# giech/usrp_nfc

Hardware: AMD Instinct MI355X
Metric: IQ Msamples/s -> decoded bits (2 Msps stream) (higher is better)
Workload: dtype f32 envelope / f64 window sums / u8 symbols; 1 GPU; configs[1]: Miller-only decode, synthetic IQ @2 Msps; input_kind=fc32 IQ, 8 B/sample (envelope computed in the kernel), samples_per_gpu=100000000, parallelism=time-chunk x1, edges_per_gpu=6627699, symbols_reader=3971547, symbols_tag=0, packets=101186, boundary_redos=0, exchange=none, stepping=sync, in_flight=1

## Files before the change

usrp_nfc_amd/csrc/decode.hip.h:

```cpp
#pragma once
#include <hip/hip_runtime.h>
#include <stdint.h>

#include "../../include/nfc_amd.h"
#include "scan.hip.h"

namespace nfc {

struct DecTables {
    const uint4 *mil_map;
    const uint2 *man_map;
    const uint16_t *mil_step;
    const uint16_t *man_step;
    int32_t nd;
    int32_t reader, tag;
    const uint2 *qmil_map;
    const uint16_t *qmil_step;
    uint32_t q_rep[2];
    uint32_t canon[4];
    int32_t q_ok;
};
__device__ __forceinline__ uint32_t byte_of(const uint32_t *w, uint32_t i) { return (w[i >> 2] >> (8u * (i & 3u))) & 0xFFu; }

struct DecCarry {
    int32_t mil_state, man_state;
    int32_t pkt_started[2];
    uint32_t pending[2];
};

constexpr int DEC_ITEMS = 16;
#ifndef NFC_DEC_GROUPS
#define NFC_DEC_GROUPS 2
#endif
constexpr int DEC_GROUPS = NFC_DEC_GROUPS;
constexpr int DEC_PER_THREAD = DEC_ITEMS * DEC_GROUPS;
constexpr int DEC_TILE = SCAN_BLOCK * DEC_PER_THREAD;
constexpr int DEC_LDS_ROWS = 512;
inline size_t dec_num_tiles(size_t n) { return (n + DEC_TILE - 1) / DEC_TILE; }

enum DecLdsUser { DEC_LDS_SPEC = 0, DEC_LDS_REDUCE = 1, DEC_LDS_APPLY = 2 };
inline size_t dec_table_bytes(DecLdsUser k, const DecTables &T) {
    const size_t rows = 4 * (size_t)T.nd, nr = T.reader ? 1 : 0, nt = T.tag ? 1 : 0;
    if (rows > (size_t)DEC_LDS_ROWS) return 0;
    switch (k) {
    case DEC_LDS_SPEC: return (nr + nt) * (rows * 16 + (rows + 1) * 8);
    case DEC_LDS_REDUCE: return nr * rows * 16 + nt * rows * 8;
    default: return nr * rows * 32 + nt * rows * 16;
    }
}

__device__ __forceinline__ void load_codes(const uint16_t *ecode, size_t base, size_t n, uint32_t (&c)[8]) {
    if (base + DEC_ITEMS <= n) {
        const uint4 a = *(const uint4 *)(ecode + base), b = *(const uint4 *)(ecode + base + 8);
        c[0] = a.x; c[1] = a.y; c[2] = a.z; c[3] = a.w;
        c[4] = b.x; c[5] = b.y; c[6] = b.z; c[7] = b.w;
    } else {
#pragma unroll
        for (int k = 0; k < 8; k++) {
            const size_t i = base + 2 * k;
            c[k] = (i < n ? (uint32_t)ecode[i] : 0u) | (i + 1 < n ? (uint32_t)ecode[i + 1] << 16 : 0u);
        }
    }
}
__device__ __forceinline__ void load_bytes16(const uint8_t *p, size_t base, size_t n, uint32_t fill, uint32_t (&w)[4]) {
    if (base + 16 <= n) {
        const uint4 a = *(const uint4 *)(p + base);
        w[0] = a.x; w[1] = a.y; w[2] = a.z; w[3] = a.w;
    } else {
#pragma unroll
        for (int k = 0; k < 4; k++) {
            uint32_t v = 0;
#pragma unroll
            for (int q = 0; q < 4; q++) {
                const size_t i = base + 4 * k + q;
                v |= (i < n ? (uint32_t)p[i] : fill) << (8 * q);
            }
            w[k] = v;
        }
    }
}

constexpr uint32_t PM_STOP = 0u, PM_START = 1u, PM_ID = 2u;
constexpr uint32_t FA_DB = 4u, FA_DC = 8u;
struct FrameAgg {
    uint32_t cnt[2];
    uint32_t nb[2], nc[2];
    uint32_t fl[2];
};
struct FrameAggOp {
    using T = FrameAgg;
    static __host__ __device__ __forceinline__ T identity() { return T{{0u, 0u}, {0u, 0u}, {0u, 0u}, {PM_ID, PM_ID}}; }
    static __device__ __forceinline__ T op(const T &a, const T &b) {
        T r;
#pragma unroll
        for (int t = 0; t < 2; t++) {
            const uint32_t ma = a.fl[t] & 3u, mb = b.fl[t] & 3u;
            const bool into_stopped = ma == PM_STOP;
            r.cnt[t] = a.cnt[t] + b.cnt[t];
            r.nb[t] = a.nb[t] + b.nb[t] - (into_stopped ? (b.fl[t] >> 2) & 1u : 0u);
            r.nc[t] = a.nc[t] + b.nc[t] - (into_stopped ? (b.fl[t] >> 3) & 1u : 0u);
            r.fl[t] = (mb == PM_ID ? ma : mb) | ((ma == PM_ID ? b.fl[t] : a.fl[t]) & (FA_DB | FA_DC));
        }
        return r;
    }
    static __device__ __forceinline__ T shfl_up(const T &v, int d) {
        T r;
#pragma unroll
        for (int t = 0; t < 2; t++) {
            r.cnt[t] = (uint32_t)__shfl_up((int)v.cnt[t], d, 64);
            r.nb[t] = (uint32_t)__shfl_up((int)v.nb[t], d, 64);
            r.nc[t] = (uint32_t)__shfl_up((int)v.nc[t], d, 64);
            r.fl[t] = (uint32_t)__shfl_up((int)v.fl[t], d, 64);
        }
        return r;
    }
};
struct FramePk {
    uint32_t a[2], b[2];
};
struct FramePkOp {
    using T = FramePk;
    static __device__ __forceinline__ T pack(const FrameAgg &f) {
        return T{{f.cnt[0] | (f.nb[0] << 16), f.cnt[1] | (f.nb[1] << 16)}, {f.nc[0] | (f.fl[0] << 16), f.nc[1] | (f.fl[1] << 16)}};
    }
    static __device__ __forceinline__ FrameAgg unpack(const T &p) {
        return FrameAgg{{p.a[0] & 0xFFFFu, p.a[1] & 0xFFFFu}, {p.a[0] >> 16, p.a[1] >> 16}, {p.b[0] & 0xFFFFu, p.b[1] & 0xFFFFu}, {p.b[0] >> 16, p.b[1] >> 16}};
    }
    static __device__ __forceinline__ T identity() { return T{{0u, 0u}, {PM_ID << 16, PM_ID << 16}}; }
    static __device__ __forceinline__ T op(const T &x, const T &y) {
        T r;
#pragma unroll
        for (int t = 0; t < 2; t++) {
            const uint32_t ma = (x.b[t] >> 16) & 3u, mb = (y.b[t] >> 16) & 3u;
            const uint32_t stopped = ma == PM_STOP ? 1u : 0u;
            r.a[t] = x.a[t] + y.a[t] - ((stopped & (y.b[t] >> 18)) << 16);
            const uint32_t nc = (x.b[t] & 0xFFFFu) + (y.b[t] & 0xFFFFu) - (stopped & (y.b[t] >> 19));
            const uint32_t fl = (mb == PM_ID ? ma : mb) | (((ma == PM_ID ? y.b[t] : x.b[t]) >> 16) & (FA_DB | FA_DC));
            r.b[t] = nc | (fl << 16);
        }
        return r;
    }
};
__device__ __forceinline__ uint32_t pm_apply(uint32_t fl, uint32_t started) { return (fl & 3u) == PM_ID ? started : (fl & 3u); }
__device__ __forceinline__ uint32_t fa_bits(const FrameAgg &a, int t, uint32_t started) { return a.nb[t] - (started ? 0u : (a.fl[t] >> 2) & 1u); }
__device__ __forceinline__ uint32_t fa_closes(const FrameAgg &a, int t, uint32_t started) { return a.nc[t] - (started ? 0u : (a.fl[t] >> 3) & 1u); }
__device__ __forceinline__ uint32_t start_bit_of(int type) { return type == 0 ? 1u : 0u; }
__device__ __forceinline__ uint32_t transpose_pairs(uint32_t m0, uint32_t m1, uint32_t m2, uint32_t m3) {
    uint32_t x = m0 | (m1 << 2) | (m2 << 4) | (m3 << 6);
    uint32_t t = (x ^ (x >> 6)) & 0x00CC00CCu;
    x ^= t ^ (t << 6);
    t = (x ^ (x >> 12)) & 0x0000F0F0u;
    x ^= t ^ (t << 12);
    return x;
}
struct SlotMasks {
    uint32_t V[2], ST[2], SA[2];
};
template <int DECS = 3>
__device__ __forceinline__ SlotMasks slot_masks(const uint32_t (&ow)[4]) {
    constexpr uint32_t M = 0x01010101u;
    uint32_t V1[4], ST1[4], SA1[4], V0[4], ST0[4], SA0[4];
#pragma unroll
    for (int i = 0; i < 4; i++) {
        const uint32_t w = ow[i];
        const uint32_t b0 = w & M, b1 = (w >> 1) & M;
        const uint32_t v0 = b0 & b1;
        const uint32_t v1e = b0 ^ b1;
        const uint32_t v1o = b1 & ~b0;
        const uint32_t c2 = (w >> 2) & M, hi0 = ((w >> 3) | (w >> 4)) & M;
        const uint32_t c5 = (w >> 5) & M, hi1 = ((w >> 6) | (w >> 7)) & M;
        const uint32_t z0 = M ^ (c2 | hi0), z1 = M ^ (c5 | hi1);
        const uint32_t o0 = c2 & ~hi0;
        V1[i] = v1e | (v1o << 1);
        ST1[i] = (hi0 & v1e) | ((hi1 & v1o) << 1);
        SA1[i] = (z0 & v1e) | ((z1 & v1o) << 1);
        V0[i] = v0;
        ST0[i] = hi0 & v0;
        SA0[i] = o0 & v0;
    }
    SlotMasks m{{0u, 0u}, {0u, 0u}, {0u, 0u}};
    if (DECS & 2) {
        m.V[0] = transpose_pairs(V0[0], V0[1], V0[2], V0[3]);
        m.ST[0] = transpose_pairs(ST0[0], ST0[1], ST0[2], ST0[3]);
        m.SA[0] = transpose_pairs(SA0[0], SA0[1], SA0[2], SA0[3]);
    }
    if (DECS & 1) {
        m.V[1] = transpose_pairs(V1[0], V1[1], V1[2], V1[3]);
        m.ST[1] = transpose_pairs(ST1[0], ST1[1], ST1[2], ST1[3]);
        m.SA[1] = transpose_pairs(SA1[0], SA1[1], SA1[2], SA1[3]);
    }
    return m;
}
__device__ __forceinline__ uint32_t started_before(const SlotMasks &m, int t, uint32_t started) {
    const uint32_t x = m.SA[t] | ~(m.ST[t] | m.SA[t]), y = m.SA[t];
    return (x + y + started) ^ x ^ y;
}
template <int DECS = 3>
__device__ __forceinline__ FrameAgg frame_agg_of(const uint32_t (&ow)[4]) {
    const SlotMasks m = slot_masks<DECS>(ow);
    FrameAgg a;
#pragma unroll
    for (int t = 0; t < 2; t++) {
        const uint32_t nonid = m.ST[t] | m.SA[t];
        const uint32_t before = started_before(m, t, 1u);
        const uint32_t appended = m.V[t] & ~m.ST[t] & (before | ~m.SA[t]);
        const uint32_t closes = m.ST[t] & before;
        const uint32_t first = nonid & (0u - nonid);
        a.cnt[t] = (uint32_t)__popc(m.V[t]);
        a.nb[t] = (uint32_t)__popc(appended);
        a.nc[t] = (uint32_t)__popc(closes);
        a.fl[t] = nonid == 0u ? PM_ID
                              : ((m.ST[t] > m.SA[t] ? PM_STOP : PM_START) | ((first & m.SA[t]) ? FA_DB : 0u) | ((first & m.ST[t]) ? FA_DC : 0u));
    }
    return a;
}
__device__ __forceinline__ uint32_t compress32(uint32_t x, uint32_t m) {
    x &= m;
    uint32_t mk = ~m << 1;
#pragma unroll
    for (int i = 0; i < 5; i++) {
        uint32_t mp = mk ^ (mk << 1);
        mp ^= mp << 2;
        mp ^= mp << 4;
        mp ^= mp << 8;
        mp ^= mp << 16;
        const uint32_t mv = mp & m;
        m = (m ^ mv) | (mv >> (1 << i));
        const uint32_t t = x & mv;
        x = (x ^ t) | (t >> (1 << i));
        mk &= ~mp;
    }
    return x;
}
__device__ __forceinline__ uint32_t symbol_low_bits(const uint32_t (&ow)[4]) {
    constexpr uint32_t M = 0x01010101u;
    uint32_t b[4];
#pragma unroll
    for (int i = 0; i < 4; i++) b[i] = ((ow[i] >> 2) & M) | (((ow[i] >> 5) & M) << 1);
    return transpose_pairs(b[0], b[1], b[2], b[3]);
}

struct PktCnt {
    uint64_t v[2];
};

struct ZeroJob {
    uint32_t *p[2];
    uint32_t n[2];
};
__device__ __forceinline__ void zero_words(const ZeroJob &Z) {
#pragma unroll
    for (int t = 0; t < 2; t++)
        for (uint32_t i = blockIdx.x * blockDim.x + threadIdx.x; i < Z.n[t]; i += gridDim.x * blockDim.x) Z.p[t][i] = 0u;
}

template <bool LDS>
__global__ __launch_bounds__(SCAN_BLOCK) void k_dec_reduce(const uint16_t *ecode, size_t n, const uint32_t *n_dev, DecTables T,
                                                          DecMaps *partials, DecMaps *aggs, ZeroJob Z) {
    zero_words(Z);
    if (n_dev) n = min(n, (size_t)*n_dev);
    if ((size_t)blockIdx.x * DEC_TILE >= n) return;
    TP_DECL();
    extern __shared__ __attribute__((aligned(16))) unsigned char s_dec_tab[];
    uint4 *const s_mil = (uint4 *)s_dec_tab;
    uint2 *const s_man = (uint2 *)(s_mil + (LDS && T.reader ? 4 * T.nd : 0));
    __shared__ DecMaps lds[SCAN_WAVES];
    if (LDS) {
        const int rows = 4 * T.nd;
        for (int i = threadIdx.x; i < rows; i += SCAN_BLOCK) {
            if (T.reader) s_mil[i] = T.mil_map[i];
            if (T.tag) s_man[i] = T.man_map[i];
        }
        __syncthreads();
    }
    const size_t tid = (size_t)blockIdx.x * SCAN_BLOCK + threadIdx.x;
    uint32_t c[DEC_GROUPS][8];
#pragma unroll
    for (int g = 0; g < DEC_GROUPS; g++) load_codes(ecode, tid * DEC_PER_THREAD + DEC_ITEMS * g, n, c[g]);
    TP_MARK();
    DecMaps agg = ComposeDec::identity();
#pragma unroll
    for (int g = 0; g < DEC_GROUPS; g++) {
#pragma unroll
        for (int k = 0; k < DEC_ITEMS; k++) {
            const uint32_t code = (c[g][k >> 1] >> (16 * (k & 1))) & 0xFFFFu;
            const uint32_t li = code & 0x3FFFu, route = code >> 14;
            if (route == 2u && T.reader) {
                const uint4 v = LDS ? s_mil[li] : T.mil_map[li];
#pragma unroll
                for (int q = 0; q < 4; q++) agg.mil[q] = lookup16x4(v.x, v.y, v.z, v.w, agg.mil[q]);
            } else if (route == 1u && T.tag) {
                const uint2 v = LDS ? s_man[li] : T.man_map[li];
                agg.man[0] = __builtin_amdgcn_perm(v.y, v.x, agg.man[0]);
                agg.man[1] = __builtin_amdgcn_perm(v.y, v.x, agg.man[1]);
            }
        }
    }
    TP_MARK();
    aggs[tid] = agg;
    DecMaps total;
    (void)block_exclusive<ComposeDec>(agg, lds, total);
    if (threadIdx.x == 0) partials[blockIdx.x] = total;
    TP_DONE(1);
}

template <bool LDS>
__global__ __launch_bounds__(SCAN_BLOCK) void k_dec_apply(const uint16_t *ecode, size_t n, const uint32_t *n_dev, DecTables T,
                                                         const DecMaps *partials, const DecMaps *aggs, uint32_t state0,
                                                         uint8_t *outw, FrameAgg *frame_aggs, FramePk *thread_aggs, bool own_prefix, DecMaps *total_out) {
    if (n_dev) n = min(n, (size_t)*n_dev);
    if (own_prefix && n == 0 && blockIdx.x == 0 && threadIdx.x == 0) *total_out = ComposeDec::identity();
    if ((size_t)blockIdx.x * DEC_TILE >= n) return;
    TP_DECL();
    extern __shared__ __attribute__((aligned(16))) unsigned char s_dec_tab[];
    uint16_t *const s_mil = (uint16_t *)s_dec_tab;
    uint16_t *const s_man = s_mil + (LDS && T.reader ? 4 * T.nd * 16 : 0);
    __shared__ DecMaps lds[SCAN_WAVES];
    __shared__ FramePk lds2[SCAN_WAVES];
    const DecMaps pre = own_prefix ? tile_prefix<ComposeDec, SCAN_BLOCK>(partials, blockIdx.x, lds) : partials[blockIdx.x];
    TP_MARK();
    if (LDS) {
        const int rows = 4 * T.nd;
        if (T.reader)
            for (int i = threadIdx.x; i < rows * 2; i += SCAN_BLOCK) ((uint4 *)s_mil)[i] = ((const uint4 *)T.mil_step)[i];
        if (T.tag)
            for (int i = threadIdx.x; i < rows; i += SCAN_BLOCK) ((uint4 *)s_man)[i] = ((const uint4 *)T.man_step)[i];
    }
    const size_t tid = (size_t)blockIdx.x * SCAN_BLOCK + threadIdx.x;
    const size_t base = tid * DEC_PER_THREAD;
    uint32_t c[DEC_GROUPS][8];
#pragma unroll
    for (int g = 0; g < DEC_GROUPS; g++) load_codes(ecode, base + DEC_ITEMS * g, n, c[g]);
    DecMaps total;
    const DecMaps excl = block_exclusive<ComposeDec>(aggs[tid], lds, total);
    if (own_prefix && threadIdx.x == 0 && ((size_t)blockIdx.x + 1) * DEC_TILE >= n) *total_out = ComposeDec::op(pre, total);
    uint32_t st = ComposeDec::step(ComposeDec::op(pre, excl), state0);
    TP_MARK();
    const uint16_t *mil = LDS ? s_mil : T.mil_step;
    const uint16_t *man = LDS ? s_man : T.man_step;
    FramePk mine = FramePkOp::identity();
#pragma unroll
    for (int g = 0; g < DEC_GROUPS; g++) {
        uint32_t ow[4] = {0u, 0u, 0u, 0u};
#pragma unroll
        for (int k = 0; k < DEC_ITEMS; k++) {
            const uint32_t code = (c[g][k >> 1] >> (16 * (k & 1))) & 0xFFFFu;
            const uint32_t li = code & 0x3FFFu, route = code >> 14;
            uint32_t w = 0;
            if (route == 2u && T.reader) {
                const uint32_t e = mil[li * 16u + (st & 15u)];
                w = e >> 8;
                st = (st & ~15u) | (e & 15u);
            } else if (route == 1u && T.tag) {
                const uint32_t e = man[li * 8u + ((st >> 4) & 7u)];
                const uint32_t m = e >> 8;
                w = (m & 3u) ? ((m & 0xFCu) | 3u) : 0u;
                st = (st & 15u) | ((e & 15u) << 4);
            }
            ow[k >> 2] |= w << (8 * (k & 3));
        }
        const size_t gb = base + (size_t)DEC_ITEMS * g;
        if (gb < n) *(uint4 *)(outw + gb) = make_uint4(ow[0], ow[1], ow[2], ow[3]);
        mine = FramePkOp::op(mine, FramePkOp::pack(frame_agg_of(ow)));
    }
    TP_MARK();
    FramePk total_fa;
    *(uint4 *)(thread_aggs + tid) = make_uint4(mine.a[0], mine.a[1], mine.b[0], mine.b[1]);
    (void)block_exclusive<FramePkOp>(mine, lds2, total_fa);
    if (threadIdx.x == 0) frame_aggs[blockIdx.x] = FramePkOp::unpack(total_fa);
    TP_DONE(2);
}

constexpr int FW_WORDS = DEC_TILE * 2 / 32 + 4;
constexpr uint32_t ST_CLOSES = 512 * DEC_GROUPS;
struct TileStage {
    uint32_t *bits[2];
    uint32_t *close_bit[2];
    uint64_t *close_idx[2];
    uint32_t *drop_bit[2];
    FrameAgg *own;
    const uint32_t *epos;
    uint64_t g0;
    const uint64_t *idx64;
};
__device__ __forceinline__ void bitcopy_or(uint32_t *dst, uint32_t dst_bit, const uint32_t *src, uint32_t src_bit, uint32_t nbits, uint32_t cap_bits) {
    if (!nbits) return;
    const uint32_t w0 = dst_bit >> 5, nw = ((dst_bit & 31u) + nbits + 31u) >> 5, capw = (cap_bits + 31u) >> 5;
    for (uint32_t j = threadIdx.x; j < nw; j += blockDim.x) {
        if (w0 + j >= capw) break;
        const uint32_t lo = max(dst_bit, (w0 + j) << 5), hi = min(dst_bit + nbits, (w0 + j + 1u) << 5);
        const uint32_t sb = src_bit + (lo - dst_bit), k = sb & 31u;
        const uint32_t a = src[sb >> 5], b = k ? src[(sb >> 5) + 1u] : 0u;
        uint32_t v = (a >> k) | (k ? b << (32u - k) : 0u);
        const uint32_t cnt = hi - lo;
        if (cnt < 32u) v &= (1u << cnt) - 1u;
        v <<= (lo & 31u);
        if (v) atomicOr(dst + w0 + j, v);
    }
}

struct QMaps {
    uint32_t mil[2];
    uint32_t man[2];
};
struct ComposeQ {
    using T = QMaps;
    static __host__ __device__ __forceinline__ T identity() { return T{{0x03020100u, 0x07060504u}, {0x03020100u, 0x07060504u}}; }
    static __device__ __forceinline__ T op(const T &a, const T &b) {
        return T{{__builtin_amdgcn_perm(b.mil[1], b.mil[0], a.mil[0]), __builtin_amdgcn_perm(b.mil[1], b.mil[0], a.mil[1])},
                 {__builtin_amdgcn_perm(b.man[1], b.man[0], a.man[0]), __builtin_amdgcn_perm(b.man[1], b.man[0], a.man[1])}};
    }
    static __device__ __forceinline__ uint32_t step(const T &m, uint32_t st) {
        const uint32_t a = __builtin_amdgcn_perm(m.mil[1], m.mil[0], st & 7u) & 15u;
        const uint32_t b = __builtin_amdgcn_perm(m.man[1], m.man[0], (st >> 4) & 7u) & 15u;
        return a | (b << 4);
    }
};
struct DecSpec {
    QMaps map;
    uint32_t s_in;
    uint32_t needs;
    uint32_t pad[2];
};
static_assert(sizeof(DecSpec) == 32, "two 16-byte loads");
__device__ __forceinline__ bool map8_constant(const uint32_t (&m)[2]) { return m[0] == m[1] && m[0] == (m[0] & 0xFFu) * 0x01010101u; }
constexpr int DEC_RUNIN_MAX = 8;
static_assert(DEC_GROUPS >= 1 && DEC_GROUPS <= 2, "NFC_DEC_GROUPS: a thread's packed bits are accumulated in 64 bits (32 slots per group)");
static_assert(DEC_RUNIN_MAX * SCAN_BLOCK <= DEC_TILE, "the longest run-in fits inside the tile before");
template <bool LDS, int DECS>
__global__ __launch_bounds__(SCAN_BLOCK) void k_dec_spec(const uint16_t *ecode, size_t n, const uint32_t *n_dev, DecTables T, uint32_t state0, int runin_per_thread,
                                                        uint8_t *outw, FrameAgg *frame_aggs, DecSpec *spec, ZeroJob Z, TileStage S) {
    constexpr bool RD = (DECS & 1) != 0, TG = (DECS & 2) != 0;
    zero_words(Z);
    if (n_dev) n = min(n, (size_t)*n_dev);
    if ((size_t)blockIdx.x * DEC_TILE >= n) return;
    TP_DECL();
    extern __shared__ __attribute__((aligned(16))) unsigned char s_dec_tab[];
    const int trows = LDS ? 4 * T.nd : 0;
    uint16_t *const s_mil = (uint16_t *)s_dec_tab, *const s_man = s_mil + (RD ? trows * 8 : 0);
    uint2 *const s_milmap = (uint2 *)(s_man + (TG ? trows * 8 : 0)), *const s_manmap = s_milmap + (LDS && RD ? trows + 1 : 0);
    __shared__ QMaps lds[SCAN_WAVES];
    __shared__ FramePk lds2[SCAN_WAVES];
    __shared__ uint32_t s_needs;
    __shared__ uint32_t s_bits[2][FW_WORDS];
    __shared__ uint32_t s_drop[2];
    for (int i = threadIdx.x; i < 2 * FW_WORDS; i += SCAN_BLOCK) (&s_bits[0][0])[i] = 0u;
    if (threadIdx.x < 2) s_drop[threadIdx.x] = 0xFFFFFFFFu;
    const uint32_t ident = 4u * (uint32_t)T.nd;
    if (LDS) {
        const int rows = 4 * T.nd;
        for (int i = threadIdx.x; i <= rows; i += SCAN_BLOCK) {
            if (RD) s_milmap[i] = T.qmil_map[i];
            if (TG) s_manmap[i] = T.man_map[i];
        }
        for (int i = threadIdx.x; i < rows; i += SCAN_BLOCK) {
            if (RD) ((uint4 *)s_mil)[i] = ((const uint4 *)T.qmil_step)[i];
            if (TG) ((uint4 *)s_man)[i] = ((const uint4 *)T.man_step)[i];
        }
    }
    if (threadIdx.x == 0) s_needs = 0u;
    const size_t tid = (size_t)blockIdx.x * SCAN_BLOCK + threadIdx.x;
    const size_t base = tid * DEC_PER_THREAD;
    uint32_t c[DEC_GROUPS][8];
#pragma unroll
    for (int g = 0; g < DEC_GROUPS; g++) load_codes(ecode, base + DEC_ITEMS * g, n, c[g]);
    uint32_t rc[DEC_RUNIN_MAX / 2];
    const bool have_runin = blockIdx.x > 0;
    {
        const size_t r0 = (size_t)blockIdx.x * DEC_TILE - (size_t)runin_per_thread * SCAN_BLOCK + (size_t)threadIdx.x * runin_per_thread;
#pragma unroll
        for (int k = 0; k < DEC_RUNIN_MAX / 2; k++) rc[k] = (have_runin && 2 * k < runin_per_thread) ? *(const uint32_t *)(ecode + r0 + 2 * k) : 0u;
    }
    __syncthreads();
    TP_MARK();
    auto mil_row = [&](uint32_t code) __attribute__((always_inline)) -> uint2 {
        const uint32_t idx = (code >> 14) == 2u ? (code & 0x3FFFu) : ident;
        return LDS ? s_milmap[idx] : T.qmil_map[idx];
    };
    auto man_row = [&](uint32_t code) __attribute__((always_inline)) -> uint2 {
        const uint32_t idx = (code >> 14) == 1u ? (code & 0x3FFFu) : ident;
        return LDS ? s_manmap[idx] : T.man_map[idx];
    };
    auto then = [](const uint2 &a, const uint2 &b) __attribute__((always_inline)) -> uint2 {
        return make_uint2(__builtin_amdgcn_perm(b.y, b.x, a.x), __builtin_amdgcn_perm(b.y, b.x, a.y));
    };
    auto routes_of = [](uint32_t pair) __attribute__((always_inline)) -> uint32_t {
        const uint32_t r0 = (pair >> 14) & 3u, r1 = pair >> 30;
        return ((r0 == 2u || r1 == 2u) ? 1u : 0u) | ((r0 == 1u || r1 == 1u) ? 2u : 0u);
    };
    auto compose4 = [&](uint2 &am, uint2 &an, uint32_t w0, uint32_t w1) __attribute__((always_inline)) {
        const uint32_t c0 = w0 & 0xFFFFu, c1 = w0 >> 16, c2 = w1 & 0xFFFFu, c3 = w1 >> 16;
        if (RD) am = then(am, then(then(mil_row(c0), mil_row(c1)), then(mil_row(c2), mil_row(c3))));
        if (TG) an = then(an, then(then(man_row(c0), man_row(c1)), then(man_row(c2), man_row(c3))));
    };
    const QMaps idm = ComposeQ::identity();
    QMaps runin = idm;
    if (have_runin) {
        uint2 am = make_uint2(idm.mil[0], idm.mil[1]), an = make_uint2(idm.man[0], idm.man[1]);
#pragma unroll
        for (int k = 0; k < DEC_RUNIN_MAX / 2; k += 2)
            if (2 * k < runin_per_thread) compose4(am, an, rc[k], rc[k + 1]);
        const QMaps ra{{am.x, am.y}, {an.x, an.y}};
        (void)block_exclusive<ComposeQ>(ra, lds, runin);
    }
    uint32_t seen = 0u;
    uint2 am = make_uint2(idm.mil[0], idm.mil[1]), an = make_uint2(idm.man[0], idm.man[1]);
#ifndef NFC_DEC_CHAIN
#define NFC_DEC_CHAIN 8
#endif
    constexpr int CHAIN = NFC_DEC_CHAIN;
    static_assert(CHAIN == 16 || CHAIN == 8 || CHAIN == 4, "NFC_DEC_CHAIN");
    constexpr int NCH = DEC_PER_THREAD / CHAIN;
    uint2 pm[NCH], pn[NCH];
#pragma unroll
    for (int g = 0; g < DEC_GROUPS; g++) {
#pragma unroll
        for (int k = 0; k < 8; k += 2) {
            if (k % (CHAIN / 2) == 0) {
                pm[(16 * g + 2 * k) / CHAIN] = am;
                pn[(16 * g + 2 * k) / CHAIN] = an;
            }
            compose4(am, an, c[g][k], c[g][k + 1]);
            seen |= routes_of(c[g][k]) | routes_of(c[g][k + 1]);
        }
    }
    if (!RD) seen &= ~1u;
    if (!TG) seen &= ~2u;
    const QMaps agg{{am.x, am.y}, {an.x, an.y}};
    TP_MARK();
    QMaps total;
    const QMaps excl = block_exclusive<ComposeQ>(agg, lds, total);
    const QMaps upto = ComposeQ::op(runin, excl);
    const uint32_t dep = ((seen & 1u) && !map8_constant(upto.mil) ? 1u : 0u) | ((seen & 2u) && !map8_constant(upto.man) ? 2u : 0u);
    if (blockIdx.x > 0 && dep) atomicOr(&s_needs, dep);
    uint32_t st[NCH];
#pragma unroll
    for (int j = 0; j < NCH; j++) st[j] = ComposeQ::step(ComposeQ::op(upto, QMaps{{pm[j].x, pm[j].y}, {pn[j].x, pn[j].y}}), state0);
    TP_MARK();
    const uint16_t *mil = LDS ? s_mil : T.qmil_step;
    const uint16_t *man = LDS ? s_man : T.man_step;
    uint32_t ow[DEC_GROUPS][4];
#pragma unroll
    for (int g = 0; g < DEC_GROUPS; g++) ow[g][0] = ow[g][1] = ow[g][2] = ow[g][3] = 0u;
#pragma unroll
    for (int e = 0; e < CHAIN; e++) {
#pragma unroll
        for (int j = 0; j < NCH; j++) {
            const int g = (j * CHAIN) / DEC_ITEMS, k = (j * CHAIN) % DEC_ITEMS + e;
            const uint32_t code = (c[g][k >> 1] >> (16 * (k & 1))) & 0xFFFFu;
            const uint32_t li = code & 0x3FFFu, route = code >> 14;
            uint32_t w = 0;
            if (route == 2u && RD) {
                const uint32_t en = mil[li * 8u + (st[j] & 7u)];
                w = en >> 8;
                st[j] = (st[j] & ~15u) | (en & 15u);
            } else if (route == 1u && TG) {
                const uint32_t en = man[li * 8u + ((st[j] >> 4) & 7u)];
                const uint32_t m = en >> 8;
                w = (m & 3u) ? ((m & 0xFCu) | 3u) : 0u;
                st[j] = (st[j] & 15u) | ((en & 15u) << 4);
            }
            ow[g][k >> 2] |= w << (8 * (k & 3));
        }
    }
    FramePk mine = FramePkOp::identity();
#pragma unroll
    for (int g = 0; g < DEC_GROUPS; g++) {
        const size_t gb = base + (size_t)DEC_ITEMS * g;
        if (gb < n) *(uint4 *)(outw + gb) = make_uint4(ow[g][0], ow[g][1], ow[g][2], ow[g][3]);
        mine = FramePkOp::op(mine, FramePkOp::pack(frame_agg_of<DECS>(ow[g])));
    }
    TP_MARK();
    FramePk total_fa;
    const FramePk in_tile = block_exclusive<FramePkOp>(mine, lds2, total_fa);
    {
        FrameAgg before = FramePkOp::unpack(in_tile);
        uint64_t acc[2] = {0ull, 0ull};
        uint32_t cnt[2] = {0u, 0u};
        const uint32_t bo0[2] = {before.nb[0], before.nb[1]};
#pragma unroll
        for (int g = 0; g < DEC_GROUPS; g++) {
            if (ow[g][0] | ow[g][1] | ow[g][2] | ow[g][3]) {
                const SlotMasks m = slot_masks<DECS>(ow[g]);
                const uint32_t low = symbol_low_bits(ow[g]);
#pragma unroll
                for (int t = 0; t < 2; t++) {
                    if (!(t ? RD : TG) || !m.V[t]) continue;
                    const uint32_t started = pm_apply(before.fl[t], 1u);
                    const uint32_t bef = started_before(m, t, started);
                    const uint32_t appended = m.V[t] & ~m.ST[t] & (bef | ~m.SA[t]);
                    uint32_t cl = m.ST[t] & bef;
                    const uint32_t bo = bo0[t] + cnt[t];
                    const uint32_t nonid = m.ST[t] | m.SA[t];
                    if ((before.fl[t] & 3u) == PM_ID && nonid) {
                        const uint32_t first = nonid & (0u - nonid);
                        if (first & m.SA[t]) s_drop[t] = bo + (uint32_t)__popc(appended & (first - 1u));
                    }
                    acc[t] |= (uint64_t)compress32(low, appended) << cnt[t];
                    cnt[t] += (uint32_t)__popc(appended);
                    if (cl) {
                        const uint32_t co = before.nc[t], closes = cl;
                        while (cl) {
                            const uint32_t lowb = cl & (0u - cl);
                            const int k = (__ffs((int)cl) - 1) >> 1;
                            cl ^= lowb;
                            const uint32_t j = co + (uint32_t)__popc(closes & (lowb - 1u));
                            if (j < ST_CLOSES) {
                                const size_t e = base + (size_t)DEC_ITEMS * g + k;
                                S.close_bit[t][(size_t)blockIdx.x * ST_CLOSES + j] = bo + (uint32_t)__popc(appended & (lowb - 1u));
                                S.close_idx[t][(size_t)blockIdx.x * ST_CLOSES + j] = S.idx64 ? S.idx64[e] : S.g0 + (uint64_t)S.epos[e];
                            } else {
                                atomicOr(&s_needs, 4u);
                            }
                        }
                    }
                }
                if (g + 1 < DEC_GROUPS) before = FrameAggOp::op(before, frame_agg_of<DECS>(ow[g]));
            }
        }
#pragma unroll
        for (int t = 0; t < 2; t++) {
            if (!cnt[t]) continue;
            const uint32_t w = bo0[t] >> 5, sh = bo0[t] & 31u;
            const uint64_t lo = acc[t] << sh;
            const uint32_t hi = sh ? (uint32_t)(acc[t] >> (64u - sh)) : 0u;
            if (w + 2 < (uint32_t)FW_WORDS) {
                if ((uint32_t)lo) atomicOr(&s_bits[t][w], (uint32_t)lo);
                if ((uint32_t)(lo >> 32)) atomicOr(&s_bits[t][w + 1], (uint32_t)(lo >> 32));
                if (hi) atomicOr(&s_bits[t][w + 2], hi);
            }
        }
    }
    __syncthreads();
    const FrameAgg tile_fa = FramePkOp::unpack(total_fa);
#pragma unroll
    for (int t = 0; t < 2; t++) {
        if (!(t ? RD : TG)) continue;
        const uint32_t nw = min((uint32_t)FW_WORDS, (tile_fa.nb[t] + 31u) / 32u + 1u);
        for (uint32_t j = threadIdx.x; j < nw; j += SCAN_BLOCK) S.bits[t][(size_t)blockIdx.x * FW_WORDS + j] = s_bits[t][j];
    }
    if (threadIdx.x == 0) {
        frame_aggs[blockIdx.x] = tile_fa;
        S.own[blockIdx.x] = tile_fa;
        if (TG) S.drop_bit[0][blockIdx.x] = s_drop[0];
        if (RD) S.drop_bit[1][blockIdx.x] = s_drop[1];
        const uint32_t s_in = ComposeQ::step(runin, state0);
        ((uint4 *)(spec + blockIdx.x))[0] = make_uint4(total.mil[0], total.mil[1], total.man[0], total.man[1]);
        ((uint4 *)(spec + blockIdx.x))[1] = make_uint4(s_in, s_needs, 0u, 0u);
    }
    TP_DONE(1);
}

using DecSpecKernel = void (*)(const uint16_t *, size_t, const uint32_t *, DecTables, uint32_t, int, uint8_t *, FrameAgg *, DecSpec *, ZeroJob, TileStage);
inline DecSpecKernel dec_spec_kernel(bool lds, const DecTables &T) {
    static const DecSpecKernel k[2][4] = {{k_dec_spec<false, 0>, k_dec_spec<false, 1>, k_dec_spec<false, 2>, k_dec_spec<false, 3>},
                                          {k_dec_spec<true, 0>, k_dec_spec<true, 1>, k_dec_spec<true, 2>, k_dec_spec<true, 3>}};
    return k[lds ? 1 : 0][(T.reader ? 1 : 0) | (T.tag ? 2 : 0)];
}

struct DecVerify {
    const DecSpec *spec;
    uint32_t state0;
    uint32_t q_rep[2];
    DecCarry *carry;
    uint32_t *verdict;
};
constexpr int DV_ITEMS = 4;
__device__ __forceinline__ void dec_verify(const DecVerify &V, size_t ntiles, QMaps *lds) {
    QMaps before = ComposeQ::identity();
    int bad = 0;
    for (size_t b0 = 0; b0 < ntiles; b0 += (size_t)SCAN_BLOCK * DV_ITEMS) {
        const size_t i0 = b0 + (size_t)threadIdx.x * DV_ITEMS;
        QMaps mp[DV_ITEMS];
        uint32_t s_in[DV_ITEMS], needs[DV_ITEMS];
#pragma unroll
        for (int k = 0; k < DV_ITEMS; k++) {
            if (i0 + k < ntiles) {
                const uint4 a = ((const uint4 *)(V.spec + i0 + k))[0], b = ((const uint4 *)(V.spec + i0 + k))[1];
                mp[k] = QMaps{{a.x, a.y}, {a.z, a.w}};
                s_in[k] = b.x;
                needs[k] = b.y;
            } else {
                mp[k] = ComposeQ::identity();
                s_in[k] = 0u;
                needs[k] = 0u;
            }
        }
        QMaps agg = mp[0];
#pragma unroll
        for (int k = 1; k < DV_ITEMS; k++) agg = ComposeQ::op(agg, mp[k]);
        QMaps total;
        QMaps run = ComposeQ::op(before, block_exclusive<ComposeQ>(agg, lds, total));
#pragma unroll
        for (int k = 0; k < DV_ITEMS; k++) {
            const uint32_t diff = ComposeQ::step(run, V.state0) ^ s_in[k];
            if (((needs[k] & 1u) && (diff & 15u)) || ((needs[k] & 2u) && (diff >> 4)) || (needs[k] & 4u)) bad = 1;
            run = ComposeQ::op(run, mp[k]);
        }
        before = ComposeQ::op(before, total);
    }
    bad = __syncthreads_or(bad);
    if (threadIdx.x == 0) {
        const uint32_t st = ComposeQ::step(before, V.state0);
        V.carry->mil_state = (int32_t)byte_of(V.q_rep, st & 7u);
        V.carry->man_state = (int32_t)(st >> 4);
        *V.verdict = bad ? 1u : 0u;
    }
}

struct FrameOut {
    uint8_t *sym[2];
    uint32_t cap_sym[2];
    const uint32_t *epos;
    uint64_t g0;
    const uint64_t *idx64;
    uint8_t *bits[2];
    uint32_t *close_end[2];
    uint64_t *close_idx[2];
    uint32_t cap_bits[2], cap_close[2];
    const uint8_t *pending[2];
    uint32_t pend[2], started_in[2];
};
__device__ __forceinline__ void copy_pending(const FrameOut &P, int tid, int nthreads) {
#pragma unroll
    for (int t = 0; t < 2; t++)
        for (uint32_t i = tid; i < P.pend[t] && i < P.cap_bits[t]; i += nthreads) P.bits[t][i] = P.pending[t][i];
}
__device__ __forceinline__ void frame_write(const FrameOut &P, const FrameAgg &pre, const uint32_t (&ow)[4], size_t base) {
    const SlotMasks m = slot_masks(ow);
    const uint64_t lo = (uint64_t)ow[0] | ((uint64_t)ow[1] << 32), hi = (uint64_t)ow[2] | ((uint64_t)ow[3] << 32);
#pragma unroll
    for (int t = 0; t < 2; t++) {
        uint32_t v = m.V[t];
        if (!v) continue;
        const uint32_t started = pm_apply(pre.fl[t], P.started_in[t]);
        const uint32_t before = started_before(m, t, started);
        const uint32_t appended = v & ~m.ST[t] & (before | ~m.SA[t]);
        const uint32_t closes = m.ST[t] & before;
        uint32_t off = pre.cnt[t];
        const uint32_t bo = P.pend[t] + fa_bits(pre, t, P.started_in[t]), co = fa_closes(pre, t, P.started_in[t]);
        if (__all(off + 33u < P.cap_sym[t] && bo + 32u < P.cap_bits[t])) {
            uint8_t *const sp = P.sym[t], *const bp = P.bits[t];
            uint32_t bi = bo;
            while (v) {
                const uint32_t low = v & (0u - v);
                const int slot = __ffs((int)v) - 1, k = slot >> 1;
                v ^= low;
                const uint32_t byte = (uint32_t)((k < 8 ? lo : hi) >> (8 * (k & 7))) & 0xFFu;
                const uint32_t s = (byte >> ((slot & 1) ? 5 : 2)) & 7u;
                sp[off++] = (uint8_t)s;
                if (appended & low) bp[bi++] = (uint8_t)s;
            }
            uint32_t cl = closes;
            while (cl) {
                const uint32_t low = cl & (0u - cl);
                const int k = (__ffs((int)cl) - 1) >> 1;
                cl ^= low;
                const uint32_t j = co + (uint32_t)__popc(closes & (low - 1u));
                if (j < P.cap_close[t]) {
                    P.close_end[t][j] = bo + (uint32_t)__popc(appended & (low - 1u));
                    P.close_idx[t][j] = P.idx64 ? P.idx64[base + k] : P.g0 + (uint64_t)P.epos[base + k];
                }
            }
            continue;
        }
        while (v) {
            const uint32_t low = v & (0u - v);
            const int slot = __ffs((int)v) - 1, k = slot >> 1;
            v ^= low;
            const uint32_t byte = (uint32_t)((k < 8 ? lo : hi) >> (8 * (k & 7))) & 0xFFu;
            const uint32_t s = (byte >> ((slot & 1) ? 5 : 2)) & 7u;
            if (off + 1 < P.cap_sym[t]) P.sym[t][off] = (uint8_t)s;
            off++;
            if (appended & low) {
                const uint32_t i = bo + (uint32_t)__popc(appended & (low - 1u));
                if (i < P.cap_bits[t]) P.bits[t][i] = (uint8_t)s;
            } else if (closes & low) {
                const uint32_t j = co + (uint32_t)__popc(closes & (low - 1u));
                if (j < P.cap_close[t]) {
                    P.close_end[t][j] = bo + (uint32_t)__popc(appended & (low - 1u));
                    P.close_idx[t][j] = P.idx64 ? P.idx64[base + k] : P.g0 + (uint64_t)P.epos[base + k];
                }
            }
        }
    }
}
struct DecCarryEpilogue {
    const DecMaps *total;
    uint32_t state_in;
    DecCarry *carry;
    uint32_t *nsym;
    PktCnt *pk_total;
    uint32_t pend[2], started_in[2];
    uint32_t canon[4];
    __device__ __forceinline__ void operator()(const FrameAgg &ft) const {
        if (total) {
            const uint32_t st = ComposeDec::step(*total, state_in);
            carry->mil_state = (int32_t)byte_of(canon, st & 15u);
            carry->man_state = (int32_t)(st >> 4);
        }
        nsym[1] = ft.cnt[1];
        nsym[0] = ft.cnt[0];
#pragma unroll
        for (int t = 0; t < 2; t++)
            pk_total->v[t] = (uint64_t)(pend[t] + fa_bits(ft, t, started_in[t])) | ((uint64_t)fa_closes(ft, t, started_in[t]) << 32);
    }
};

__device__ __forceinline__ void pack_pending(const FrameOut &P, int tid, int nthreads) {
#pragma unroll
    for (int t = 0; t < 2; t++) {
        if (!P.bits[t]) continue;
        uint32_t *gb = (uint32_t *)P.bits[t];
        for (uint32_t i = tid; i < P.pend[t] && i < P.cap_bits[t]; i += nthreads)
            if (P.pending[t][i] & 1u) atomicOr(gb + (i >> 5), 1u << (i & 31));
    }
}
__global__ __launch_bounds__(SCAN_BLOCK) void k_frame_write(const uint8_t *outw, size_t n, const uint32_t *n_dev, const FrameAgg *tile_pre,
                                                           const FramePk *thread_aggs, FrameOut P, bool own_prefix, FrameAgg *total_out,
                                                           DecCarryEpilogue epi, DecVerify V) {
    if (n_dev) n = min(n, (size_t)*n_dev);
    if (V.spec) {
        if (blockIdx.x == 0) {
            __shared__ QMaps lds_v[SCAN_WAVES];
            dec_verify(V, (n + DEC_TILE - 1) / DEC_TILE, lds_v);
            return;
        }
    }
    const uint32_t bid = blockIdx.x - (V.spec ? 1u : 0u);
    if (bid == 0) pack_pending(P, threadIdx.x, SCAN_BLOCK);
    if (own_prefix && n == 0 && bid == 0 && threadIdx.x == 0) {
        *total_out = FrameAggOp::identity();
        epi(FrameAggOp::identity());
    }
    if ((size_t)bid * DEC_TILE >= n) return;
    TP_DECL();
    __shared__ FramePk lds[SCAN_WAVES];
    __shared__ FrameAgg lds_pre[SCAN_WAVES];
    __shared__ uint32_t s_bits[2][FW_WORDS];
    for (int i = threadIdx.x; i < 2 * FW_WORDS; i += SCAN_BLOCK) (&s_bits[0][0])[i] = 0u;
    const FrameAgg pre = own_prefix ? tile_prefix<FrameAggOp, SCAN_BLOCK>(tile_pre, bid, lds_pre) : tile_pre[bid];
    const size_t base = ((size_t)bid * SCAN_BLOCK + threadIdx.x) * DEC_PER_THREAD;
    TP_MARK();
    uint32_t ow[DEC_GROUPS][4];
#pragma unroll
    for (int g = 0; g < DEC_GROUPS; g++) {
        ow[g][0] = ow[g][1] = ow[g][2] = ow[g][3] = 0u;
        const size_t gb = base + (size_t)DEC_ITEMS * g;
        if (gb < n) {
            const uint4 a = *(const uint4 *)(outw + gb);
            ow[g][0] = a.x; ow[g][1] = a.y; ow[g][2] = a.z; ow[g][3] = a.w;
        }
    }
    const uint4 m4 = *(const uint4 *)(thread_aggs + (size_t)bid * SCAN_BLOCK + threadIdx.x);
    FramePk total;
    const FramePk in_tile = block_exclusive<FramePkOp>(FramePk{{m4.x, m4.y}, {m4.z, m4.w}}, lds, total);
    const FrameAgg all = FrameAggOp::op(pre, FramePkOp::unpack(total));
    if (own_prefix && threadIdx.x == 0 && ((size_t)bid + 1) * DEC_TILE >= n) {
        *total_out = all;
        epi(all);
    }
    TP_MARK();
    FrameAgg before = FrameAggOp::op(pre, FramePkOp::unpack(in_tile));
    uint64_t acc[2] = {0ull, 0ull};
    uint32_t cnt[2] = {0u, 0u}, bo0[2], tile_bit0[2];
#pragma unroll
    for (int t = 0; t < 2; t++) {
        bo0[t] = P.pend[t] + fa_bits(before, t, P.started_in[t]);
        tile_bit0[t] = P.pend[t] + fa_bits(pre, t, P.started_in[t]);
    }
#pragma unroll
    for (int g = 0; g < DEC_GROUPS; g++) {
        if (ow[g][0] | ow[g][1] | ow[g][2] | ow[g][3]) {
            const SlotMasks m = slot_masks(ow[g]);
            const uint32_t low = symbol_low_bits(ow[g]);
#pragma unroll
            for (int t = 0; t < 2; t++) {
                if (!m.V[t] || !P.bits[t]) continue;
                const uint32_t started = pm_apply(before.fl[t], P.started_in[t]);
                const uint32_t bef = started_before(m, t, started);
                const uint32_t appended = m.V[t] & ~m.ST[t] & (bef | ~m.SA[t]);
                uint32_t cl = m.ST[t] & bef;
                const uint32_t bo = bo0[t] + cnt[t];
                acc[t] |= (uint64_t)compress32(low, appended) << cnt[t];
                cnt[t] += (uint32_t)__popc(appended);
                if (cl) {
                    const uint32_t co = fa_closes(before, t, P.started_in[t]);
                    const uint32_t closes = cl;
                    while (cl) {
                        const uint32_t lowb = cl & (0u - cl);
                        const int k = (__ffs((int)cl) - 1) >> 1;
                        cl ^= lowb;
                        const uint32_t j = co + (uint32_t)__popc(closes & (lowb - 1u));
                        if (j < P.cap_close[t]) {
                            P.close_end[t][j] = bo + (uint32_t)__popc(appended & (lowb - 1u));
                            const size_t e = base + (size_t)DEC_ITEMS * g + k;
                            P.close_idx[t][j] = P.idx64 ? P.idx64[e] : P.g0 + (uint64_t)P.epos[e];
                        }
                    }
                }
            }
            if (g + 1 < DEC_GROUPS) before = FrameAggOp::op(before, frame_agg_of(ow[g]));
        }
    }
#pragma unroll
    for (int t = 0; t < 2; t++) {
        if (!cnt[t]) continue;
        const uint32_t lb = (tile_bit0[t] & 31u) + (bo0[t] - tile_bit0[t]);
        const uint32_t w = lb >> 5, sh = lb & 31u;
        const uint64_t lo = acc[t] << sh;
        const uint32_t hi = sh ? (uint32_t)(acc[t] >> (64u - sh)) : 0u;
        if (w + 2 < (uint32_t)FW_WORDS) {
            if ((uint32_t)lo) atomicOr(&s_bits[t][w], (uint32_t)lo);
            if ((uint32_t)(lo >> 32)) atomicOr(&s_bits[t][w + 1], (uint32_t)(lo >> 32));
            if (hi) atomicOr(&s_bits[t][w + 2], hi);
        }
    }
    TP_MARK();
    __syncthreads();
#pragma unroll
    for (int t = 0; t < 2; t++) {
        if (!P.bits[t]) continue;
        const uint32_t nbits = P.pend[t] + fa_bits(all, t, P.started_in[t]) - tile_bit0[t];
        if (!nbits) continue;
        uint32_t *gb = (uint32_t *)P.bits[t];
        const uint32_t w0 = tile_bit0[t] >> 5, nw = ((tile_bit0[t] & 31u) + nbits + 31u) >> 5, capw = (P.cap_bits[t] + 31u) >> 5;
        for (uint32_t j = threadIdx.x; j < nw; j += SCAN_BLOCK) {
            if (w0 + j >= capw) break;
            const uint32_t v = s_bits[t][j];
            if (j == 0 || j == nw - 1) atomicOr(gb + w0 + j, v);
            else gb[w0 + j] = v;
        }
    }
    TP_DONE(3);
}

__global__ __launch_bounds__(SCAN_BLOCK) void k_concat(size_t n, const uint32_t *n_dev, const FrameAgg *tile_pre, TileStage S, FrameOut P, bool own_prefix,
                                                      FrameAgg *total_out, DecCarryEpilogue epi, DecVerify V) {
    if (n_dev) n = min(n, (size_t)*n_dev);
    if (blockIdx.x == 0) {
        __shared__ QMaps lds_v[SCAN_WAVES];
        dec_verify(V, (n + DEC_TILE - 1) / DEC_TILE, lds_v);
        return;
    }
    const uint32_t bid = blockIdx.x - 1u;
    if (bid == 0) pack_pending(P, threadIdx.x, SCAN_BLOCK);
    if (own_prefix && n == 0 && bid == 0 && threadIdx.x == 0) {
        *total_out = FrameAggOp::identity();
        epi(FrameAggOp::identity());
    }
    if ((size_t)bid * DEC_TILE >= n) return;
    TP_DECL();
    __shared__ FrameAgg lds_pre[SCAN_WAVES];
    const FrameAgg pre = own_prefix ? tile_prefix<FrameAggOp, SCAN_BLOCK>(tile_pre, bid, lds_pre) : tile_pre[bid];
    const FrameAgg own = S.own[bid];
    TP_MARK();
    if (own_prefix && threadIdx.x == 0 && ((size_t)bid + 1) * DEC_TILE >= n) {
        const FrameAgg all = FrameAggOp::op(pre, own);
        *total_out = all;
        epi(all);
    }
#pragma unroll
    for (int t = 0; t < 2; t++) {
        if (!P.bits[t] || !S.bits[t]) continue;
        const uint32_t started = pm_apply(pre.fl[t], P.started_in[t]);
        const uint32_t bit0 = P.pend[t] + fa_bits(pre, t, P.started_in[t]);
        const uint32_t nb = own.nb[t];
        const bool drop = !started && (own.fl[t] & FA_DB);
        const uint32_t q = drop ? S.drop_bit[t][bid] : 0xFFFFFFFFu;
        const uint32_t *src = S.bits[t] + (size_t)bid * FW_WORDS;
        uint32_t *dst = (uint32_t *)P.bits[t];
        if (!drop) {
            bitcopy_or(dst, bit0, src, 0u, nb, P.cap_bits[t]);
        } else if (q < nb) {
            bitcopy_or(dst, bit0, src, 0u, q, P.cap_bits[t]);
            bitcopy_or(dst, bit0 + q, src, q + 1u, nb - 1u - q, P.cap_bits[t]);
        }
        const bool dropc = !started && (own.fl[t] & FA_DC);
        const uint32_t ncl = min(own.nc[t], ST_CLOSES), co = fa_closes(pre, t, P.started_in[t]);
        for (uint32_t i = threadIdx.x; i < ncl; i += SCAN_BLOCK) {
            if (dropc && i == 0) continue;
            const uint32_t j = co + i - (dropc ? 1u : 0u);
            if (j >= P.cap_close[t]) continue;
            const uint32_t e = S.close_bit[t][(size_t)bid * ST_CLOSES + i];
            P.close_end[t][j] = bit0 + e - ((drop && e > q) ? 1u : 0u);
            P.close_idx[t][j] = S.close_idx[t][(size_t)bid * ST_CLOSES + i];
        }
    }
    TP_DONE(3);
}

__global__ __launch_bounds__(SCAN_BLOCK) void k_symbols_write(const uint8_t *outw, size_t n, const uint32_t *n_dev, const FrameAgg *tile_pre,
                                                             FrameOut P, bool own_prefix) {
    if (n_dev) n = min(n, (size_t)*n_dev);
    if ((size_t)blockIdx.x * DEC_TILE >= n) return;
    __shared__ FramePk lds[SCAN_WAVES];
    __shared__ FrameAgg lds_pre[SCAN_WAVES];
    const FrameAgg pre = own_prefix ? tile_prefix<FrameAggOp, SCAN_BLOCK>(tile_pre, blockIdx.x, lds_pre) : tile_pre[blockIdx.x];
    const size_t base = ((size_t)blockIdx.x * SCAN_BLOCK + threadIdx.x) * DEC_PER_THREAD;
    uint32_t owa[DEC_GROUPS][4];
    FramePk mine = FramePkOp::identity();
#pragma unroll
    for (int g = 0; g < DEC_GROUPS; g++) {
        owa[g][0] = owa[g][1] = owa[g][2] = owa[g][3] = 0u;
        const size_t gb = base + (size_t)DEC_ITEMS * g;
        if (gb < n) {
            const uint4 a = *(const uint4 *)(outw + gb);
            owa[g][0] = a.x; owa[g][1] = a.y; owa[g][2] = a.z; owa[g][3] = a.w;
        }
        mine = FramePkOp::op(mine, FramePkOp::pack(frame_agg_of(owa[g])));
    }
    FramePk total;
    const FramePk in_tile = block_exclusive<FramePkOp>(mine, lds, total);
    FrameAgg before = FrameAggOp::op(pre, FramePkOp::unpack(in_tile));
#pragma unroll
    for (int g = 0; g < DEC_GROUPS; g++) {
        const size_t gb = base + (size_t)DEC_ITEMS * g;
        if (gb >= n) break;
        const uint32_t ow[4] = {owa[g][0], owa[g][1], owa[g][2], owa[g][3]};
        if (!(ow[0] | ow[1] | ow[2] | ow[3])) continue;
        const SlotMasks m = slot_masks(ow);
        const uint64_t lo = (uint64_t)ow[0] | ((uint64_t)ow[1] << 32), hi = (uint64_t)ow[2] | ((uint64_t)ow[3] << 32);
#pragma unroll
        for (int t = 0; t < 2; t++) {
            uint32_t v = m.V[t], off = before.cnt[t];
            while (v) {
                const int slot = __ffs((int)v) - 1, k = slot >> 1;
                v &= v - 1u;
                const uint32_t byte = (uint32_t)((k < 8 ? lo : hi) >> (8 * (k & 7))) & 0xFFu;
                if (off + 1 < P.cap_sym[t]) P.sym[t][off] = (uint8_t)((byte >> ((slot & 1) ? 5 : 2)) & 7u);
                off++;
            }
        }
        before = FrameAggOp::op(before, frame_agg_of(ow));
    }
}

struct PktFinish {
    const uint8_t *bits[2];
    uint8_t *pending_next[2];
    const uint32_t *close_end[2];
    const PktCnt *totals;
    const FrameAgg *frame_total;
    DecCarry *carry;
    int32_t enabled[2], started_in[2];
    uint32_t pending_cap[2];
    uint32_t cap_bits[2], cap_close[2];
    const uint32_t *mirror_src;
    uint32_t *mirror_dst;
    uint32_t mirror_words;
    uint32_t stamp_word, stamp;
    int32_t packed;
};
__global__ __launch_bounds__(256) void k_pkt_finish(PktFinish F) {
    for (int t = 0; t < 2; t++) {
        if (!F.enabled[t]) continue;
        const uint64_t tot = F.totals->v[t];
        const uint32_t nbits = (uint32_t)tot, ncl = (uint32_t)(tot >> 32);
        if (nbits > F.cap_bits[t] || ncl > F.cap_close[t]) continue;
        const uint32_t from = ncl ? F.close_end[t][ncl - 1] : 0u;
        const uint32_t keep = nbits - from;
        const uint32_t *bw = (const uint32_t *)F.bits[t];
        for (uint32_t i = threadIdx.x; i < keep && i < F.pending_cap[t]; i += blockDim.x)
            F.pending_next[t][i] = F.packed ? (uint8_t)((bw[(from + i) >> 5] >> ((from + i) & 31u)) & 1u) : F.bits[t][from + i];
        if (threadIdx.x == 0) {
            F.carry->pending[t] = keep;
            F.carry->pkt_started[t] = (int32_t)pm_apply(F.frame_total->fl[t], (uint32_t)F.started_in[t]);
        }
    }
    if (F.mirror_src) {
        __threadfence_block();
        __syncthreads();
        for (uint32_t i = threadIdx.x; i < F.mirror_words; i += blockDim.x)
            if (i != F.stamp_word) F.mirror_dst[i] = F.mirror_src[i];
        __threadfence_system();
        __syncthreads();
        if (threadIdx.x == 0) {
            ((volatile uint32_t *)F.mirror_dst)[F.stamp_word] = F.stamp;
        }
    }
}

}
```

Before: 457,600 Msamples/s.

## Prefetch codes and tables early, branchless decode step, defer zeroing in k_dec_spec

Issues the global loads for the code words, run-in codes and LDS table rows at kernel entry, before the n_dev check and the LDS initialisation, so their latency overlaps setup work. Boundary masking of the codes is applied only to tail threads. The per-symbol decode replaces route branches with mask-based selects and splits each step into a batched table-lookup phase and an update phase. Zeroing of the scratch words moves to the end of the kernel, and per-variant waves_per_eu occupancy hints are added. This risks higher register pressure and out-of-range speculative loads being clamped via min.

```diff
diff --git a/usrp_nfc_amd/csrc/decode.hip.h b/usrp_nfc_amd/csrc/decode.hip.h
--- a/usrp_nfc_amd/csrc/decode.hip.h
+++ b/usrp_nfc_amd/csrc/decode.hip.h
@@ -60,6 +60,19 @@
             const size_t i = base + 2 * k;
             c[k] = (i < n ? (uint32_t)ecode[i] : 0u) | (i + 1 < n ? (uint32_t)ecode[i + 1] << 16 : 0u);
         }
+    }
+}
+__device__ __forceinline__ void request_codes(const uint16_t *ecode, size_t base, size_t cap, uint32_t (&c)[8]) {
+    const size_t last = cap & ~(size_t)7;
+    const uint4 a = *(const uint4 *)(ecode + min(base, last)), b = *(const uint4 *)(ecode + min(base + 8, last));
+    c[0] = a.x; c[1] = a.y; c[2] = a.z; c[3] = a.w;
+    c[4] = b.x; c[5] = b.y; c[6] = b.z; c[7] = b.w;
+}
+__device__ __forceinline__ void mask_codes(size_t base, size_t n, uint32_t (&c)[8]) {
+#pragma unroll
+    for (int k = 0; k < 8; k++) {
+        const size_t i = base + 2 * k;
+        c[k] &= (i < n ? 0xFFFFu : 0u) | (i + 1 < n ? 0xFFFF0000u : 0u);
     }
 }
 __device__ __forceinline__ void load_bytes16(const uint8_t *p, size_t base, size_t n, uint32_t fill, uint32_t (&w)[4]) {
@@ -248,10 +261,11 @@
     uint32_t *p[2];
     uint32_t n[2];
 };
+template <int BLOCK = SCAN_BLOCK>
 __device__ __forceinline__ void zero_words(const ZeroJob &Z) {
 #pragma unroll
     for (int t = 0; t < 2; t++)
-        for (uint32_t i = blockIdx.x * blockDim.x + threadIdx.x; i < Z.n[t]; i += gridDim.x * blockDim.x) Z.p[t][i] = 0u;
+        for (uint32_t i = blockIdx.x * BLOCK + threadIdx.x; i < Z.n[t]; i += gridDim.x * BLOCK) Z.p[t][i] = 0u;
 }
 
 template <bool LDS>
@@ -428,12 +442,9 @@
 static_assert(DEC_GROUPS >= 1 && DEC_GROUPS <= 2, "NFC_DEC_GROUPS: a thread's packed bits are accumulated in 64 bits (32 slots per group)");
 static_assert(DEC_RUNIN_MAX * SCAN_BLOCK <= DEC_TILE, "the longest run-in fits inside the tile before");
 template <bool LDS, int DECS>
-__global__ __launch_bounds__(SCAN_BLOCK) void k_dec_spec(const uint16_t *ecode, size_t n, const uint32_t *n_dev, DecTables T, uint32_t state0, int runin_per_thread,
+__global__ __launch_bounds__(SCAN_BLOCK) __attribute__((amdgpu_waves_per_eu(DECS == 3 ? 4 : (LDS && DECS != 0) ? 5 : 1))) void k_dec_spec(const uint16_t *ecode, size_t n, const uint32_t *n_dev, DecTables T, uint32_t state0, int runin_per_thread,
                                                         uint8_t *outw, FrameAgg *frame_aggs, DecSpec *spec, ZeroJob Z, TileStage S) {
     constexpr bool RD = (DECS & 1) != 0, TG = (DECS & 2) != 0;
-    zero_words(Z);
-    if (n_dev) n = min(n, (size_t)*n_dev);
-    if ((size_t)blockIdx.x * DEC_TILE >= n) return;
     TP_DECL();
     extern __shared__ __attribute__((aligned(16))) unsigned char s_dec_tab[];
     const int trows = LDS ? 4 * T.nd : 0;
@@ -444,26 +455,22 @@
     __shared__ uint32_t s_needs;
     __shared__ uint32_t s_bits[2][FW_WORDS];
     __shared__ uint32_t s_drop[2];
-    for (int i = threadIdx.x; i < 2 * FW_WORDS; i += SCAN_BLOCK) (&s_bits[0][0])[i] = 0u;
-    if (threadIdx.x < 2) s_drop[threadIdx.x] = 0xFFFFFFFFu;
-    const uint32_t ident = 4u * (uint32_t)T.nd;
+    uint32_t n_now = 0xFFFFFFFFu;
+    if (n_dev) {
+        uint32_t zero = 0u;
+        asm volatile("" : "+v"(zero));
+        n_now = n_dev[zero];
+    }
+    uint2 rm = {}, rn = {};
+    uint4 wm = {}, wn = {};
     if (LDS) {
-        const int rows = 4 * T.nd;
-        for (int i = threadIdx.x; i <= rows; i += SCAN_BLOCK) {
-            if (RD) s_milmap[i] = T.qmil_map[i];
-            if (TG) s_manmap[i] = T.man_map[i];
-        }
-        for (int i = threadIdx.x; i < rows; i += SCAN_BLOCK) {
-            if (RD) ((uint4 *)s_mil)[i] = ((const uint4 *)T.qmil_step)[i];
-            if (TG) ((uint4 *)s_man)[i] = ((const uint4 *)T.man_step)[i];
-        }
-    }
-    if (threadIdx.x == 0) s_needs = 0u;
+        const int im = min((int)threadIdx.x, trows), iw = min(im, trows - 1);
+        if (RD) rm = T.qmil_map[im], wm = ((const uint4 *)T.qmil_step)[iw];
+        if (TG) rn = T.man_map[im], wn = ((const uint4 *)T.man_step)[iw];
+    }
+    __builtin_amdgcn_sched_barrier(0);
     const size_t tid = (size_t)blockIdx.x * SCAN_BLOCK + threadIdx.x;
     const size_t base = tid * DEC_PER_THREAD;
-    uint32_t c[DEC_GROUPS][8];
-#pragma unroll
-    for (int g = 0; g < DEC_GROUPS; g++) load_codes(ecode, base + DEC_ITEMS * g, n, c[g]);
     uint32_t rc[DEC_RUNIN_MAX / 2];
     const bool have_runin = blockIdx.x > 0;
     {
@@ -471,8 +478,44 @@
 #pragma unroll
         for (int k = 0; k < DEC_RUNIN_MAX / 2; k++) rc[k] = (have_runin && 2 * k < runin_per_thread) ? *(const uint32_t *)(ecode + r0 + 2 * k) : 0u;
     }
+    uint32_t c[DEC_GROUPS][8];
+#pragma unroll
+    for (int g = 0; g < DEC_GROUPS; g++) request_codes(ecode, base + DEC_ITEMS * g, n, c[g]);
+    __builtin_amdgcn_sched_barrier(0);
+    for (int i = threadIdx.x; i < 2 * FW_WORDS; i += SCAN_BLOCK) (&s_bits[0][0])[i] = 0u;
+    if (threadIdx.x < 2) s_drop[threadIdx.x] = 0xFFFFFFFFu;
+    if (threadIdx.x == 0) s_needs = 0u;
+    const uint32_t ident = 4u * (uint32_t)T.nd;
+    n = min(n, (size_t)__builtin_amdgcn_readfirstlane(n_now));
+    if ((size_t)blockIdx.x * DEC_TILE >= n) {
+        zero_words<SCAN_BLOCK>(Z);
+        return;
+    }
+    if (LDS) {
+        const int i = threadIdx.x;
+        if (i <= trows) {
+            if (RD) s_milmap[i] = rm;
+            if (TG) s_manmap[i] = rn;
+        }
+        if (i < trows) {
+            if (RD) ((uint4 *)s_mil)[i] = wm;
+            if (TG) ((uint4 *)s_man)[i] = wn;
+        }
+        for (int j = i + SCAN_BLOCK; j <= trows; j += SCAN_BLOCK) {
+            if (RD) s_milmap[j] = T.qmil_map[j];
+            if (TG) s_manmap[j] = T.man_map[j];
+            if (j < trows) {
+                if (RD) ((uint4 *)s_mil)[j] = ((const uint4 *)T.qmil_step)[j];
+                if (TG) ((uint4 *)s_man)[j] = ((const uint4 *)T.man_step)[j];
+            }
+        }
+    }
     __syncthreads();
     TP_MARK();
+    if (base + DEC_PER_THREAD > n) {
+#pragma unroll
+        for (int g = 0; g < DEC_GROUPS; g++) mask_codes(base + DEC_ITEMS * g, n, c[g]);
+    }
     auto mil_row = [&](uint32_t code) __attribute__((always_inline)) -> uint2 {
         const uint32_t idx = (code >> 14) == 2u ? (code & 0x3FFFu) : ident;
         return LDS ? s_milmap[idx] : T.qmil_map[idx];
@@ -533,33 +576,48 @@
     const QMaps upto = ComposeQ::op(runin, excl);
     const uint32_t dep = ((seen & 1u) && !map8_constant(upto.mil) ? 1u : 0u) | ((seen & 2u) && !map8_constant(upto.man) ? 2u : 0u);
     if (blockIdx.x > 0 && dep) atomicOr(&s_needs, dep);
-    uint32_t st[NCH];
-#pragma unroll
-    for (int j = 0; j < NCH; j++) st[j] = ComposeQ::step(ComposeQ::op(upto, QMaps{{pm[j].x, pm[j].y}, {pn[j].x, pn[j].y}}), state0);
-    TP_MARK();
-    const uint16_t *mil = LDS ? s_mil : T.qmil_step;
-    const uint16_t *man = LDS ? s_man : T.man_step;
+    uint32_t sm[NCH], sn[NCH];
+#pragma unroll
+    for (int j = 0; j < NCH; j++) {
+        const uint32_t s = ComposeQ::step(ComposeQ::op(upto, QMaps{{pm[j].x, pm[j].y}, {pn[j].x, pn[j].y}}), state0);
+        sm[j] = s & 7u;
+        sn[j] = (s >> 4) & 7u;
+    }
+    TP_MARK();
+    const uint16_t *const mil = LDS ? s_mil : T.qmil_step;
+    const uint16_t *const man = LDS ? s_man : T.man_step;
+    const uint32_t TAB_MAN = RD ? (uint32_t)trows * 8u : 0u;
     uint32_t ow[DEC_GROUPS][4];
 #pragma unroll
     for (int g = 0; g < DEC_GROUPS; g++) ow[g][0] = ow[g][1] = ow[g][2] = ow[g][3] = 0u;
+    auto route_mask = [&](int g, int k, int bit) __attribute__((always_inline)) -> uint32_t {
+        return (uint32_t)((int32_t)(c[g][k >> 1] << (31 - bit - 16 * (k & 1))) >> 31);
+    };
 #pragma unroll
     for (int e = 0; e < CHAIN; e++) {
+        uint32_t en[NCH];
 #pragma unroll
         for (int j = 0; j < NCH; j++) {
             const int g = (j * CHAIN) / DEC_ITEMS, k = (j * CHAIN) % DEC_ITEMS + e;
             const uint32_t code = (c[g][k >> 1] >> (16 * (k & 1))) & 0xFFFFu;
-            const uint32_t li = code & 0x3FFFu, route = code >> 14;
-            uint32_t w = 0;
-            if (route == 2u && RD) {
-                const uint32_t en = mil[li * 8u + (st[j] & 7u)];
-                w = en >> 8;
-                st[j] = (st[j] & ~15u) | (en & 15u);
-            } else if (route == 1u && TG) {
-                const uint32_t en = man[li * 8u + ((st[j] >> 4) & 7u)];
-                const uint32_t m = en >> 8;
-                w = (m & 3u) ? ((m & 0xFCu) | 3u) : 0u;
-                st[j] = (st[j] & 15u) | ((en & 15u) << 4);
-            }
+            const uint32_t row = (code & 0x3FFFu) * 8u;
+            const uint32_t mtg = (RD && TG) ? route_mask(g, k, 14) : 0u;
+            const uint32_t s = (RD && TG) ? (sm[j] ^ ((sm[j] ^ sn[j]) & mtg)) : RD ? sm[j] : sn[j];
+            if (DECS == 0)
+                en[j] = 0u;
+            else if (LDS)
+                en[j] = mil[(TAB_MAN & mtg) + row + s];
+            else
+                en[j] = ((RD && TG) ? (mtg ? man : mil) : RD ? mil : man)[row + s];
+        }
+#pragma unroll
+        for (int j = 0; j < NCH; j++) {
+            const int g = (j * CHAIN) / DEC_ITEMS, k = (j * CHAIN) % DEC_ITEMS + e;
+            const uint32_t mrd = RD ? route_mask(g, k, 15) : 0u, mtg = TG ? route_mask(g, k, 14) : 0u;
+            const uint32_t m = en[j] >> 8, nx = en[j] & 7u;
+            const uint32_t w = (m & mrd) | (((m & 3u) ? ((m & 0xFCu) | 3u) : 0u) & mtg);
+            if (RD) sm[j] ^= (sm[j] ^ nx) & mrd;
+            if (TG) sn[j] ^= (sn[j] ^ nx) & mtg;
             ow[g][k >> 2] |= w << (8 * (k & 3));
         }
     }
@@ -648,6 +706,7 @@
         ((uint4 *)(spec + blockIdx.x))[0] = make_uint4(total.mil[0], total.mil[1], total.man[0], total.man[1]);
         ((uint4 *)(spec + blockIdx.x))[1] = make_uint4(s_in, s_needs, 0u, 0u);
     }
+    zero_words<SCAN_BLOCK>(Z);
     TP_DONE(1);
 }
 
```

Result: no change. 457,100 Msamples/s (-0.1%).
